# imcbrearty/GENIE

Measured on AMD Instinct MI355X. Metric: picks/sec through GCN_Detection_Network_extended.forward_fixed_source (GCS_Network.forward), higher is better.
Workload: dtype f32

## Files before the change

### genie_amd/_lib.py

```python
import ctypes
import os
import subprocess

_HERE = os.path.dirname(os.path.abspath(__file__))
REPO = os.path.dirname(_HERE)
SRC = os.path.join(_HERE, "csrc", "genie_hip.hip")
LIB_DIR = os.path.join(_HERE, "lib")
LIB_PATH = os.environ.get("GENIE_LIB_PATH", os.path.join(LIB_DIR, "libgenie_hip.so"))
INCLUDE = os.path.join(REPO, "include")

_c = ctypes
_P = _c.c_void_p
SYMBOLS = [
    ("genie_version", _c.c_int, []),
    ("genie_last_error", _c.c_char_p, []),
    ("genie_ctx_create", _c.c_int, [_c.POINTER(_P), _c.c_int, _c.c_int, _c.c_int, _P, _P, _P, _P, _P, _c.c_float]),
    ("genie_ctx_create_subgraph", _c.c_int, [_c.POINTER(_P), _c.c_int, _c.c_int, _c.c_int64, _P, _P, _P, _P, _P, _P, _P, _P, _c.c_float]),
    ("genie_ctx_destroy", _c.c_int, [_P]),
    ("genie_pool_stats", _c.c_int, [_c.c_int, _c.POINTER(_c.c_int64), _c.POINTER(_c.c_int64), _c.POINTER(_c.c_int64)]),
    ("genie_set_scale_t", _c.c_int, [_P, _c.c_float]),
    ("genie_set_edge_features", _c.c_int, [_P, _P, _P, _P]),
    ("genie_set_absolute_pos", _c.c_int, [_P, _P, _P, _P]),
    ("genie_nbr_mean", _c.c_int, [_P, _P, _P, _P, _P, _c.c_int, _P]),
    ("genie_nbr_mean_bwd", _c.c_int, [_P, _P, _P, _P, _P, _c.c_int, _P]),
    ("genie_prelu_bwd", _c.c_int, [_P, _P, _P, _c.c_int64, _P, _P, _P, _P]),
    ("genie_linear_bwd_scratch_floats", _c.c_int64, [_c.c_int]),
    ("genie_linear_bwd_wb", _c.c_int, [_P, _P, _c.c_int64, _c.c_int, _c.c_int, _P, _P, _P, _P]),
    ("genie_set_slot", _c.c_int, [_P, _c.c_int]),
    ("genie_set_station_order", _c.c_int, [_P, _P]),
    ("genie_set_phase_types", _c.c_int, [_P, _c.c_int]),
    ("genie_set_sign_input", _c.c_int, [_P, _c.c_int]),
    ("genie_set_stage2_workmap", _c.c_int, [_P, _c.c_int]),
    ("genie_set_subgraph_stations", _c.c_int, [_P, _P, _P]),
    ("genie_set_tail_precision", _c.c_int, [_P, _c.c_int]),
    ("genie_set_stage_precision", _c.c_int, [_P, _c.c_int]),
    ("genie_stage_precision", _c.c_int, [_P, _c.POINTER(_c.c_int), _c.POINTER(_c.c_int), _c.POINTER(_c.c_float), _c.POINTER(_c.c_float), _P]),
    ("genie_input_range", _c.c_int, [_P, _c.POINTER(_c.c_float), _c.POINTER(_c.c_float), _c.c_int]),
    ("genie_index_flags", _c.c_int, [_P, _c.POINTER(_c.c_uint), _c.c_int]),
    ("genie_index_check", _c.c_int, [_P, _P, _c.c_int64, _c.c_int64, _c.c_int64, _c.c_uint, _P]),
    ("genie_set_static_edge_attr", _c.c_int, [_P, _P, _P]),
    ("genie_tail_batched", _c.c_int, [_P, _c.c_int, _c.c_int, _P, _P, _P, _c.c_int, _c.c_int, _P, _c.c_int, _P, _P, _P, _P, _P]),
    ("genie_readout_grid", _c.c_int, [_P, _P, _P, _c.c_int, _P, _P]),
    ("genie_readout_query", _c.c_int, [_P, _P, _P, _P, _P, _c.c_int, _c.c_int, _P, _c.c_int, _P, _P, _P]),
    ("genie_readouts", _c.c_int, [_P, _P, _P, _P, _P, _c.c_int, _c.c_int, _P, _c.c_int, _P, _P, _P, _P]),
    ("genie_readout_grid_latent", _c.c_int, [_P, _P, _P, _c.c_int, _P, _P, _P]),
    ("genie_readout_query_latent", _c.c_int, [_P, _P, _P, _P, _P, _c.c_int, _c.c_int, _P, _c.c_int, _P, _P, _P, _P]),
    ("genie_weights_count", _c.c_int, []),
    ("genie_weights_name", _c.c_char_p, [_c.c_int]),
    ("genie_weights_numel", _c.c_int64, [_c.c_int]),
    ("genie_weights_offset", _c.c_int64, [_c.c_int]),
    ("genie_weights_blob_floats", _c.c_int64, []),
    ("genie_weights_set", _c.c_int, [_P, _c.c_char_p, _P, _c.c_int64, _P]),
    ("genie_weights_set_blob", _c.c_int, [_P, _P, _c.c_int64, _P]),
    ("genie_weights_commit", _c.c_int, [_P, _P]),
    ("genie_workspace_bytes", _c.c_size_t, [_P]),
# ... 161 lines not shown
```

### genie_amd/csrc/genie_hip.hip

```cpp
#include <hip/hip_runtime.h>
#include <stdint.h>
#include <stdio.h>
#include <stdlib.h>
#include <string.h>

#include <algorithm>
#include <array>
#include <map>
#include <memory>
#include <mutex>
#include <utility>
#include <type_traits>
#include <string>
#include <vector>

#include "genie_hip.h"
#include "s2u_plan.hpp"

#define GENIE_LD_STREAM(ptr) (*(ptr))
#define GENIE_S2_WAVES 2
#define GENIE_H2_DEPTH 6

namespace {

typedef float f32x4 __attribute__((ext_vector_type(4)));

thread_local std::string g_err;

int fail(int code, const std::string& msg) {
    g_err = msg;
    return code;
}

#define HIP_TRY(expr)                                                                              \
    do {                                                                                           \
        hipError_t e_ = (expr);                                                                    \
        if (e_ != hipSuccess)                                                                      \
            return fail(GENIE_ERR_HIP, std::string(#expr) + ": " + hipGetErrorString(e_));         \
    } while (0)
#define GENIE_TRY(expr)                                                                            \
// ... 1092 lines not shown
    int abs_ts_order;
    bool pcsr;
    bool pcsr_h2;
    DevBuf<int32_t> p_sta_rowptr, p_sta_col, p_src_rowptr, p_src_col, seg_rowptr;
    DevBuf<int32_t> p_src_of;
    DevBuf<int32_t> p_sta_of;
    DevBuf<float> mpos_sta, mpos_src, ebias_sta, ebias_src;
    bool has_edges;
    DevBuf<int32_t> sta_perm, sta_inv, sta_rowptr_p, sta_col_p;
    DevBuf<int32_t> sta_ident;
    DevBuf<float> ebias_sta_p;
    const float* ea_user;
    DevBuf<int32_t> src_tab;
    DevBuf<float> packed_h2;
    hipStream_t side_stream;
    hipEvent_t ev_fork, ev_join;
    int device = 0;
    int num_cu;
    int seg, bpc1, bpc2;
    int ks_uni, kp_uni;
    int use_fast;
    int bpc2o;
    int s2_wgmap;
    int bpc1b;
    int use_h2;
    int prec_mode;
    bool range_ok;
    float range_act, range_w;
    DevBuf<float> d_range; float* h_range;
    unsigned* h_inflag;
    struct S2uTables { DevBuf<S2uBlock> blocks; DevBuf<int32_t> xcd0; int nblk, ngroups; };
    std::map<std::pair<int, int>, S2uTables> s2u;
    std::vector<int32_t> tab_host;
    DevBuf<float> packed_s2h;
    DevBuf<unsigned> ea_frag, ea_frag_tmp;
    RowLayout s1_layout;
    std::vector<const void*> lds_attr_done;
    int xs_sta_order;
    int sign_input;
    int no_phase;
    int tail_f32;
    size_t o_xs, o_mm, o_c, o_wu, o_wv, o_part, o_sa0, o_sa1, o_bip, o_gpart, o_pj0, o_pj1, o_cv, ws_floats;
    size_t slot_stride;
    size_t big_stride;
    int tail_cu_ro, tail_cu_sa;
    int slot;
// ... 1004 lines not shown
    }
    return fail(GENIE_ERR_ARG, std::string("genie_weights_set: unknown parameter ") + name);
}

int64_t genie_weights_offset(int i) { init_registry(); return (i >= 0 && i < W_COUNT) ? g_params[i].off : -1; }
int64_t genie_weights_blob_floats(void) { init_registry(); return g_raw_total; }

int genie_weights_set_blob(genie_ctx* c, const float* blob_dev, int64_t n_floats, void* stream) {
    if (!c || !blob_dev) return fail(GENIE_ERR_ARG, "genie_weights_set_blob: null argument");
    if (n_floats != g_raw_total) return fail(GENIE_ERR_ARG, "genie_weights_set_blob: wrong blob size");
    HIP_TRY(hipMemcpyAsync(c->raw, blob_dev, sizeof(float) * n_floats, hipMemcpyDeviceToDevice, (hipStream_t)stream));
    c->dirty = true;
    return GENIE_OK;
}

int genie_weights_commit(genie_ctx* c, void* stream) {
    if (!c) return fail(GENIE_ERR_ARG, "null context");
    return ensure_packed(c, (hipStream_t)stream);
}

size_t genie_workspace_bytes(const genie_ctx* c) { return c ? c->ws_floats * sizeof(float) : 0; }

namespace {
extern "C++" template <bool PCSR>
void launch_stage1_h2(const DaArgs& a, bool abs, bool edges, bool big, int grid, hipStream_t st) {
    if (abs) {
        if (big) k_stage1_h2<8, 15, false, true, true, PCSR><<<grid, H2_THREADS, 0, st>>>(a);
        else k_stage1_h2<8, 15, false, false, true, PCSR><<<grid, H2_THREADS, 0, st>>>(a);
    } else if (edges) {
        if (big) k_stage1_h2<8, 15, true, true, false, PCSR><<<grid, H2_THREADS, 0, st>>>(a);
        else k_stage1_h2<8, 15, true, false, false, PCSR><<<grid, H2_THREADS, 0, st>>>(a);
    } else {
        if (big) k_stage1_h2<8, 15, false, true, false, PCSR><<<grid, H2_THREADS, 0, st>>>(a);
        else k_stage1_h2<8, 15, false, false, false, PCSR><<<grid, H2_THREADS, 0, st>>>(a);
    }
}

int alloc_abs_pieces(genie_ctx* c, size_t n_sta_rows, size_t n_src_rows) {
    DevBuf<unsigned> ts, tg;
    HIP_TRY(ts.alloc(4 * n_sta_rows));
    HIP_TRY(tg.alloc(4 * n_src_rows));
    c->abs_ts = std::move(ts); c->abs_tg = std::move(tg);
    return GENIE_OK;
}

int run_stage1(genie_ctx* c, const StageCall& call, const float* slice, const float* mask, float* dbg_h0, float* dbg_h1, void* ws,
               void* stream, int gi_begin, int gi_end, bool do_split) {
    int rc = check_ws(c, ws);
    if (rc) return rc;
    if (!slice || !mask) return fail(GENIE_ERR_ARG, "genie_da_stage1: null input");
    if (gi_begin < 0 || gi_end > c->G || gi_begin > gi_end) return fail(GENIE_ERR_ARG, "genie_da_stage1: bad source-node range");
    const bool whole = gi_begin == 0 && gi_end == c->G;
    if (!whole && c->pcsr) return fail(GENIE_ERR_STATE, "genie_da_stage1_range: not available on an irregular product graph");
    hipStream_t st = (hipStream_t)stream;
    if ((rc = ensure_packed(c, st))) return rc;
    const StageRoutes r = stage_routes(c, call, gi_begin, gi_end, false, false);
    const bool so = sta_order_on(c, call);
// ... 39 lines not shown
        k_stage1<true><<<(int)std::max<long long>(8, gw / 8 * 8), 256, 0, st>>>(a);
        break;
    }
    case S1Route::H2: {
        unsigned* xs = (unsigned*)((float*)ws + c->o_xs);
        const bool presplit = (c->xs_slice == slice && c->xs_mask == mask && c->xs_ws == ws && c->xs_sta_order == (so ? 1 : 0)) || !do_split;
        if (do_split) { c->xs_slice = c->xs_mask = nullptr; c->xs_ws = nullptr; }
        float* mmw = (float*)ws + c->o_mm + (c->slot % GENIE_NBIG) * c->big_stride;
        if (presplit && do_split && so && c->xs_mm_copy != c->slot % GENIE_NBIG) {
            HIP_TRY(hipMemcpyAsync(mmw, (const float*)ws + c->o_mm + c->xs_mm_copy * c->big_stride, sizeof(float) * (size_t)c->P_ext,
                                   hipMemcpyDeviceToDevice, st));
        }
        if (!presplit) {
            if (so && c->S <= SPLIT_G_MAXS) {
                HIP_TRY(hipFuncSetAttribute((const void*)k_split_rows_g, hipFuncAttributeMaxDynamicSharedMemorySize, SPLIT_G_MAXS * 32));
                k_split_rows_g<<<(unsigned)(c->P_ext / c->S), 256, (size_t)c->S * 32, st>>>(slice, mask, c->S, xs, c->sta_perm, mmw, c->P_ext,
                                                                                            input_limit(c), c->h_inflag);
            } else
                k_split_rows<<<(unsigned)((c->P_ext + 255) / 256), 256, 0, st>>>(slice, mask, c->P_ext, xs, so ? c->sta_perm : nullptr, c->S,
                                                                                mmw, input_limit(c), c->h_inflag);
        }
        a.xs = xs; a.packed = c->packed_h2; a.xs_plane = c->P_ext * (long long)XPC;
        a.np = r.layout == RowLayout::NodePlanar ? 1 : 0;
        const int grid = da_grid_w(c, (n_tiles + 1) / 2, c->bpc1b, H2_THREADS / 64);
        if (!n_tiles) break;
        if (c->abs_sta && (c->abs_dirty || !c->abs_ts || c->abs_ts_order != (so ? 1 : 0))) {
            if (!c->abs_ts) GENIE_TRY(alloc_abs_pieces(c, (size_t)c->S, (size_t)c->G_ext));
            k_abs_pieces<<<(c->S + 255) / 256, 256, 0, st>>>(c->abs_sta, so ? c->sta_perm : nullptr, c->S, c->abs_ts);
            k_abs_pieces<<<(c->G_ext + 255) / 256, 256, 0, st>>>(c->abs_src, nullptr, c->G_ext, c->abs_tg);
            c->abs_dirty = false; c->abs_ts_order = so ? 1 : 0;
            a.abs_ts = c->abs_ts; a.abs_tg = c->abs_tg;
        }
        launch_stage1_h2<false>(a, c->abs_sta != nullptr, c->has_edges, c->P_ext * XROW >= (1ll << 32), grid, st);
        break;
    }
    }
    HIP_TRY(hipGetLastError());
    if (dbg_tmp) {
        if (dbg_h0) k_permute_sta_rows<<<(unsigned)((c->P * 30 + 255) / 256), 256, 0, st>>>(dbg_tmp, c->P, 30, c->sta_perm, c->S, dbg_h0);
        if (dbg_h1) k_permute_sta_rows<<<(unsigned)((c->P * 60 + 255) / 256), 256, 0, st>>>(dbg_tmp + c->P * 30, c->P, 60, c->sta_perm, c->S, dbg_h1);
        HIP_TRY(hipStreamSynchronize(st));
    }
    return GENIE_OK;
}
}

int genie_da_stage1(genie_ctx* c, const float* slice, const float* mask, void* ws, void* stream) {
    if (!c) return fail(GENIE_ERR_ARG, "null context");
    return run_stage1(c, kInference, slice, mask, nullptr, nullptr, ws, stream, 0, c->G, true);
}

int genie_da_stage1_range(genie_ctx* c, const float* slice, const float* mask, int gi_begin, int gi_end, int first, void* ws,
                          void* stream) {
    if (!c) return fail(GENIE_ERR_ARG, "null context");
    return run_stage1(c, kInference, slice, mask, nullptr, nullptr, ws, stream, gi_begin, gi_end, first != 0);
}
// ... 2113 lines not shown
        return fail(GENIE_ERR_ARG, "genie_subgraph_csr_fill: bad argument");
    if (n_prod == 0) return GENIE_OK;
    k_subgraph_csr<true><<<(unsigned)((n_prod + 255) / 256), 256, 0, (hipStream_t)stream>>>(
        pair_sta, pair_src, n_prod, seg_rowptr, sta_rowptr, sta_col, src_rowptr, src_col, nullptr, nullptr, p_sta_rowptr, p_src_rowptr,
        p_sta_col, p_src_col);
    HIP_TRY(hipGetLastError());
    return GENIE_OK;
}

int genie_set_phase_types(genie_ctx* c, int use_phase_types) {
    if (!c) return fail(GENIE_ERR_ARG, "genie_set_phase_types: null context");
    c->no_phase = use_phase_types ? 0 : 1;
    return GENIE_OK;
}

int genie_set_subgraph_stations(genie_ctx* c, const int32_t* sta_of_prod, void* stream) {
    if (!c || !sta_of_prod) return fail(GENIE_ERR_ARG, "genie_set_subgraph_stations: null argument");
    if (!c->pcsr) return fail(GENIE_ERR_STATE, "genie_set_subgraph_stations: the context is a Cartesian product graph (station = p % n_sta)");
    if (!c->p_sta_of) HIP_TRY(c->p_sta_of.alloc((size_t)c->P));
    HIP_TRY(hipMemcpyAsync(c->p_sta_of, sta_of_prod, sizeof(int32_t) * (size_t)c->P, hipMemcpyDeviceToDevice, (hipStream_t)stream));
    return GENIE_OK;
}

int genie_set_stage2_workmap(genie_ctx* c, int blocks_of_four) {
    if (!c) return fail(GENIE_ERR_ARG, "genie_set_stage2_workmap: null context");
    c->s2_wgmap = blocks_of_four < 0 ? (c->S >= 1024) : (blocks_of_four != 0);
    return GENIE_OK;
}

int genie_set_sign_input(genie_ctx* c, int use_sign_input) {
    if (!c) return fail(GENIE_ERR_ARG, "genie_set_sign_input: null context");
    c->sign_input = use_sign_input ? 1 : 0;
    return GENIE_OK;
}

int genie_set_tail_precision(genie_ctx* c, int fp64_chains) {
    if (!c) return fail(GENIE_ERR_ARG, "genie_set_tail_precision: null context");
    c->tail_f32 = fp64_chains ? 0 : 1;
    return GENIE_OK;
}

int genie_set_stage_precision(genie_ctx* c, int mode) {
    if (!c || mode < 0 || mode > 2) return fail(GENIE_ERR_ARG, "genie_set_stage_precision: mode must be 0 (auto), 1 (f16x2) or 2 (fp32)");
    c->prec_mode = mode;
    c->xs_slice = c->xs_mask = nullptr; c->xs_ws = nullptr;
    return GENIE_OK;
// ... 65 lines not shown
```

### genie_amd/csrc/stage_kernels.hpp

```cpp

template <int N>
__device__ __forceinline__ void mma_blocks(f32x4 (&acc)[N], const f32x4 (&w)[N], const f32x4 x) {
#pragma unroll
    for (int r = 0; r < 4; ++r) {
#pragma unroll
        for (int k = 0; k < N; ++k) acc[k] = MFMA16(w[k][r], x[r], acc[k]);
    }
}

__device__ __forceinline__ void stage1_dense(const DaArgs& a, const f32x4* lw, const float* lbias, int lane, int q,
                                             bool valid, long long p, int g, int sc, float mq, f32x4 x0, f32x4 x1, f32x4 n1a,
                                             f32x4 n1b, f32x4 n2a, f32x4 n2b, float a1, float a21, float a22) {
    if (a.dbg_h0 != nullptr && valid) {
#pragma unroll
        for (int r = 0; r < 4; ++r) {
            a.dbg_h0[p * 30 + 4 * q + r] = x0[r];
            if (16 + 4 * q + r < 30) a.dbg_h0[p * 30 + 16 + 4 * q + r] = x1[r];
        }
    }
    f32x4 acc[4], w4[4];
#pragma unroll
    for (int k = 0; k < 4; ++k) acc[k] = *(const f32x4*)(lbias + (2 + k) * 16 + 4 * q);
    if (a.eb_sta != nullptr) {
#pragma unroll
// ... 342 lines not shown
        const f32x4 t = *(const f32x4*)(lbias + blk * 32 + 8 * b + 4 * h);
        y[4 * b] = t.x; y[4 * b + 1] = t.y; y[4 * b + 2] = t.z; y[4 * b + 3] = t.w;
    }
    return y;
}
__device__ __forceinline__ void h2_save32(float* __restrict__ save, long long Pn, int blk0, long long p, int h, const f32x16& v) {
#pragma unroll
    for (int m = 0; m < 4; ++m) {
        f32x4 o = {v[4 * m], v[4 * m + 1], v[4 * m + 2], v[4 * m + 3]};
        if (m == 3 && h == 1) { o.z = 0.f; o.w = 0.f; }
        *(f32x4*)(save + ((size_t)(blk0 + (m >> 1)) * Pn + p) * 16 + 8 * (m & 1) + 4 * h) = o;
    }
}
template <int K_>
__device__ __forceinline__ int row_bcast(int v) { return __builtin_amdgcn_update_dpp(0, v, 0x150 + K_, 0xf, 0xf, false); }
__device__ __forceinline__ int row_bcast_dyn(int v, int k) {
    switch (k) {
        case 0: return row_bcast<0>(v); case 1: return row_bcast<1>(v); case 2: return row_bcast<2>(v); case 3: return row_bcast<3>(v);
        case 4: return row_bcast<4>(v); case 5: return row_bcast<5>(v); case 6: return row_bcast<6>(v); case 7: return row_bcast<7>(v);
        case 8: return row_bcast<8>(v); case 9: return row_bcast<9>(v); case 10: return row_bcast<10>(v); case 11: return row_bcast<11>(v);
        case 12: return row_bcast<12>(v); case 13: return row_bcast<13>(v); case 14: return row_bcast<14>(v); default: return row_bcast<15>(v);
    }
}
template <int KS_>
__device__ __forceinline__ void split8h(const f32x16& v, u32x4 (&p)[3], unsigned sixteenth) {
#pragma unroll
    for (int d = 0; d < 4; ++d) {
        const float a = v[8 * KS_ + 2 * d], b = v[8 * KS_ + 2 * d + 1];
        const unsigned p0 = cvt_pk_f16(a, b);
        p[0][d] = p0;
        p[1][d] = cvt_pk_f16(sub_f16_lo(a, p0), sub_f16_hi(b, p0));
        p[2][d] = pk_mul_f16(p0, sixteenth);
    }
}
template <int N>
__device__ __forceinline__ void mma3(f32x16 (&acc)[N], const f32x4* lw, const int (&f0)[N], int lane, const u32x4 (&b)[3]) {
    f32x4 w[N][2];
#pragma unroll
    for (int k = 0; k < N; ++k)
#pragma unroll
        for (int p = 0; p < 2; ++p) w[k][p] = lw[(f0[k] + p) * 64 + lane];
    constexpr int WP[3] = {0, 1, 0}, BP[3] = {1, 2, 0};
#pragma unroll
    for (int t = 0; t < 3; ++t)
#pragma unroll
        for (int k = 0; k < N; ++k) acc[k] = MFMA32H(w[k][WP[t]], b[BP[t]], acc[k]);
}

#ifndef GENIE_S1_NT_C
#define GENIE_S1_NT_C 1
#endif
__device__ __forceinline__ void h2_store_c(f32x4* p, f32x4 v) {
#if GENIE_S1_NT_C
    __builtin_nontemporal_store(v, p);
#else
    *p = v;
#endif
}

template <int KS, int KP, bool EDGES, bool BIG, bool ABS = false, bool PCSR = false>
__global__ __launch_bounds__(H2_THREADS) void k_stage1_h2(DaArgs a) {
    typedef typename std::conditional<BIG, unsigned long long, unsigned>::type off_t_;
    constexpr int NF4 = H2_IMG_FLOATS / 4;
    __shared__ f32x4 lw[NF4];
    for (int i = threadIdx.x; i < NF4; i += H2_THREADS) lw[i] = ((const f32x4*)a.packed)[i];
    __syncthreads();
    const float* lbias = (const float*)(lw + H2_FRAGS * 64);
    const float* lscal = lbias + H2_NBIAS * 32;
    const float a0 = lscal[0], a1 = lscal[3], a21 = lscal[4], a22 = lscal[5];
    const float s11 = compose_slopes(a0, lscal[1]), s12 = compose_slopes(a0, lscal[2]);
    const float inf = __builtin_inff();
    const float sel0 = a0 <= 1.f ? inf : -inf, sel1 = a1 <= 1.f ? inf : -inf;
    const float sel21 = a21 <= 1.f ? inf : -inf, sel22 = a22 <= 1.f ? inf : -inf;
    const float al1 = (1.f + s11) / (32.f * KS), be1 = (1.f - s11) / (32.f * KS);
    const float al2 = (1.f + s12) / (32.f * KP), be2 = (1.f - s12) / (32.f * KP);
    const unsigned c16 = __builtin_amdgcn_readfirstlane(H2_SIXTEENTH);

    int lane = threadIdx.x & 63;
    const int wave = __builtin_amdgcn_readfirstlane(threadIdx.x >> 6);
    const int h = lane >> 5, half = (lane >> 4) & 1, jj = lane & 15;
    const bool hi = h != 0;
    const int S = a.S;
    ItemIter w(a.G, a.T, a.seg, a.nxcd, wave, a.gi0);
    const char* xs = (const char*)a.xs;
    const off_t_ la = hi ? (off_t_)a.xs_plane : (off_t_)0;
    const off_t_ gstride = (off_t_)((unsigned)S * (unsigned)XPC);

    const f32x4 fa0 = lw[(H2_FA + 0) * 64 + lane], fa1 = lw[(H2_FA + 1) * 64 + lane];
    f32x4 fp0, fp1;
    if (ABS) { fp0 = lw[(H2_FABS + 0) * 64 + lane]; fp1 = lw[(H2_FABS + 1) * 64 + lane]; }
    const unsigned tp_h = (unsigned)h * 8u;
    typedef unsigned u32x2 __attribute__((ext_vector_type(2)));
    f32x16 biasA = bias16(lbias, 0, h);
#pragma unroll
    for (int r = 0; r < 16; ++r) biasA[r] *= 16.f;

    int jt = jj;
    auto fetch_ids = [&](long long pit_, int& idv_, int& sc_, bool& valid_, int (&sta_)[KS]) {
        int gi0, tb0, gi1, tb1;
        w.decode(2 * pit_, gi0, tb0);
        const bool second = 2 * pit_ + 1 < w.nitems;
        w.decode(second ? 2 * pit_ + 1 : 2 * pit_, gi1, tb1);
        idv_ = a.src_tab[(half ? gi1 : gi0) * 16 + jt];
        const int s = (half ? tb1 : tb0) * 16 + jt;
        valid_ = s < S && (second || !half);
        sc_ = s < S ? s : S - 1;
        load_sta_ids<KS>(a.sta_col, sc_, sta_);
    };
    constexpr int KPP = PCSR ? KP : 1;
    auto fetch_pcsr = [&](long long pit_, long long& p_, bool& valid_, int (&sta_)[KS], int (&src_)[KPP], int& ds_, int& dp_) {
        const long long pr = ptile_at(a.ptile, pit_) * 32 + (lane & 31);
        valid_ = pr < a.Pn;
        p_ = valid_ ? pr : a.Pn - 1;
        const int eb = a.sta_rowptr[p_], fb = a.src_rowptr[p_];
        ds_ = a.sta_rowptr[p_ + 1] - eb;
        dp_ = a.src_rowptr[p_ + 1] - fb;
#pragma unroll
        for (int q = 0; q < KS; ++q) {
            const int v = a.sta_col[max(eb + min(q, ds_ - 1), 0)];
            sta_[q] = q < ds_ ? v : (int)p_;
        }
#pragma unroll
        for (int q = 0; q < KPP; ++q) {
            const int v = a.src_col[max(fb + min(q, dp_ - 1), 0)];
            src_[q] = q < dp_ ? v : (int)p_;
        }
    };
    int idv = 0, sc = 0, sta_id[KS], src_id[KPP], dgs = 0, dgp = 0;
    long long pcur = 0;
    bool valid = false;
    PtileIter ptw(PCSR ? (a.Pn + 31) / 32 : 0, H2_THREADS / 64, wave);
    const long long pit0 = PCSR ? ptw.i : w.it;
    const long long pstride = PCSR ? ptw.stride : w.stride;
    const long long pend = PCSR ? ptw.end : (w.nitems + 1) / 2;
    if (pit0 < pend) {
        if constexpr (PCSR) fetch_pcsr(pit0, pcur, valid, sta_id, src_id, dgs, dgp);
        else fetch_ids(pit0, idv, sc, valid, sta_id);
    }
    for (long long pit = pit0, pnext = 0; pit < pend; pit = pnext) {
        asm volatile("" : "+v"(lane));
        const int g = PCSR ? 0 : row_bcast<0>(idv);
        const long long p = PCSR ? pcur : (long long)g * S + sc;
        const off_t_ gbase0 = PCSR ? (off_t_)(unsigned long long)p * (off_t_)XPC : (off_t_)(unsigned)g * gstride;
        const unsigned sbase0 = PCSR ? 0u : (unsigned)sc * (unsigned)XPC;
        off_t_ gbase = gbase0 + la;
        off_t_ sbase = (off_t_)sbase0 + la;
        const int srcv = idv;
        float alS = 0.f, beS = 0.f, alP = 0.f, beP = 0.f;
        if constexpr (PCSR) {
            const float is = 1.f / (float)max(dgs, 1), ip = 1.f / (float)max(dgp, 1);
            alS = (1.f + s11) * 0.03125f * is; beS = (1.f - s11) * 0.03125f * is;
            alP = (1.f + s12) * 0.03125f * ip; beP = (1.f - s12) * 0.03125f * ip;
        }

        constexpr int NU = 1 + KS + KP;
        static_assert(NU % 2 == 0, "units are processed in pairs");
        constexpr int DEPTH = ABS ? 4 : GENIE_H2_DEPTH;
        u32x4 buf[NU];
        u32x2 tp[NU], tso, tgo;
        if (ABS) {
            tso = *(const u32x2*)((const char*)a.abs_ts + (tp_h + (unsigned)(PCSR ? (int)p : sc) * 16u));
            tgo = *(const u32x2*)((const char*)a.abs_tg + (tp_h + (unsigned)(PCSR ? (int)p : g) * 16u));
        }
        auto issue = [&](int u) {
            off_t_ off;
            if (u == 0) off = gbase + sbase0;
            else if (PCSR) off = (off_t_)(unsigned)(u <= KS ? sta_id[u - 1] : src_id[(u - KS - 1) % KPP]) * (off_t_)XPC + la;
            else if (u <= KS) off = gbase + (unsigned)sta_id[u - 1] * (unsigned)XPC;
            else {
                const unsigned nb = (unsigned)row_bcast_dyn(srcv, u - KS);
                off = (BIG ? (off_t_)nb * gstride : (off_t_)__umul24(nb, (unsigned)gstride)) + sbase;
            }
            if (ABS && u > 0) {
                if (u <= KS) tp[u] = *(const u32x2*)((const char*)a.abs_ts + (tp_h + (unsigned)sta_id[u - 1] * 16u));
                else if (PCSR) tp[u] = *(const u32x2*)((const char*)a.abs_tg + (tp_h + (unsigned)src_id[(u - KS - 1) % KPP] * 16u));
                else tp[u] = *(const u32x2*)((const char*)a.abs_tg + (tp_h + (unsigned)row_bcast_dyn(srcv, u - KS) * 16u));
            }
            buf[u] = *(const u32x4*)(xs + off);
        };
        const u32x4 own0 = *(const u32x4*)(xs + (gbase0 + sbase0));
#pragma unroll
        for (int u = 0; u < DEPTH; ++u) issue(u);

        f32x16 sn, h0;
        u32x4 h0p[2][3], n1p[2][3], n2p[2][3];
        unsigned m01[3], m23[3];
#pragma unroll
        for (int u = 0; u < NU; u += 2) {
#pragma unroll
            for (int d = 0; d < 2; ++d)
                if (u + DEPTH + d < NU) issue(u + DEPTH + d);
            asm volatile("" : "+v"(buf[u]), "+v"(buf[u + 1]));
            f32x16 z0, z1;
            if (ABS) {
                auto posb = [&](int uu) {
                    return uu == 0 ? u32x4{tso.x, tso.y, tgo.x, tgo.y}
                                   : uu <= KS ? u32x4{tp[uu].x, tp[uu].y, tgo.x, tgo.y} : u32x4{tso.x, tso.y, tp[uu].x, tp[uu].y};
                };
                const u32x4 p0 = posb(u), p1 = posb(u + 1);
// ... 22 lines not shown
                    m01[0] = own0.z;   m23[0] = own0.w;
                    m01[1] = buf[0].z; m23[1] = buf[0].w;
                    m01[2] = pk_mul_f16(own0.z, c16); m23[2] = pk_mul_f16(own0.w, c16);
                } else {
                    float al = uu <= KS ? al1 : al2, be = uu <= KS ? be1 : be2;
                    if constexpr (PCSR) {
                        const bool present = uu <= KS ? uu - 1 < dgs : uu - KS - 1 < dgp;
                        al = present ? (uu <= KS ? alS : alP) : 0.f;
                        be = present ? (uu <= KS ? beS : beP) : 0.f;
                    }
                    if (uu == 1 || uu == KS + 1) {
#pragma unroll
                        for (int r = 0; r < 16; ++r) sn[r] = fmaf(be, __builtin_fabsf(z[r]), al * z[r]);
                    } else {
#pragma unroll
                        for (int r = 0; r < 16; ++r) sn[r] = fmaf(be, __builtin_fabsf(z[r]), fmaf(al, z[r], sn[r]));
                    }
                }
                if (uu == KS) { split8h<0>(sn, n1p[0], c16); split8h<1>(sn, n1p[1], c16); }
                if (uu == NU - 1) { split8h<0>(sn, n2p[0], c16); split8h<1>(sn, n2p[1], c16); }
            }
            asm volatile("" : "+v"(sn), "+v"(gbase), "+v"(sbase), "+v"(jt));
        }
        int idv_n = 0, sc_n = 0, sta_n[KS], src_n[KPP], dgs_n = 0, dgp_n = 0;
        long long p_n = 0;
        bool valid_n = false;
#pragma unroll
        for (int k = 0; k < KS; ++k) sta_n[k] = 0;
#pragma unroll
        for (int k = 0; k < KPP; ++k) src_n[k] = 0;
        pnext = pit + pstride;
        const bool has_next = pnext < pend;
        if (has_next) {
            if constexpr (PCSR) fetch_pcsr(pnext, p_n, valid_n, sta_n, src_n, dgs_n, dgp_n);
            else fetch_ids(pnext, idv_n, sc_n, valid_n, sta_n);
        }
        if (a.dbg_h0 != nullptr && valid) {
#pragma unroll
            for (int r = 0; r < 16; ++r) {
                const int ch = 8 * (r >> 2) + 4 * h + (r & 3);
                if (ch < 30) a.dbg_h0[p * 30 + ch] = h0[r];
            }
        }
        split8h<0>(h0, h0p[0], c16);
        split8h<1>(h0, h0p[1], c16);
#pragma unroll
        for (int q = 0; q < 3; ++q) {
            h0p[1][q].w = hi ? m01[q] : h0p[1][q].w;
            n1p[1][q].w = hi ? m23[q] : n1p[1][q].w;
            n2p[1][q].w = hi ? m23[q] : n2p[1][q].w;
        }
        f32x16 acc[2] = {bias16(lbias, 1, h), bias16(lbias, 2, h)};
        if (EDGES) {
#pragma unroll
            for (int b = 0; b < 4; ++b) {
                const f32x4 es = *(const f32x4*)(a.eb_sta + (PCSR ? p : (long long)sc) * 48 + 8 * b + 4 * h);
                const f32x4 eg = *(const f32x4*)(a.eb_src + (PCSR ? p : (long long)g) * 48 + 8 * b + 4 * h);
#pragma unroll
// ... 78 lines not shown
            else { split8h<1>(o3[0], up, c16); split8h<1>(o3[1], vp, c16); }
            f32x4 wa[2], wb[2];
#pragma unroll
            for (int q = 0; q < 2; ++q) {
                wa[q] = lw[(H2_FW + (0 + kb) * 2 + q) * 64 + lane];
                wb[q] = lw[(H2_FW + (2 + kb) * 2 + q) * 64 + lane];
            }
            constexpr int WP[3] = {0, 1, 0}, BP[3] = {1, 2, 0};
#pragma unroll
            for (int t = 0; t < 3; ++t) {
                ow[0] = MFMA32H(wa[WP[t]], up[BP[t]], ow[0]);
                ow[1] = MFMA32H(wb[WP[t]], vp[BP[t]], ow[1]);
            }
        }
        if (valid) {
            float* vr = a.np ? a.wv + npb * ROWW + (long long)h * npl + (long long)sc * 4 : a.wv + p * ROWW + 4 * h;
            const long long vs = a.np ? 2 * npl : 8;
#pragma unroll
            for (int b = 0; b < 2; ++b) {
                *(f32x4*)(a.wu + p * ROWW + 8 * b + 4 * h) = f32x4{ow[0][4 * b], ow[0][4 * b + 1], ow[0][4 * b + 2], ow[0][4 * b + 3]};
                *(f32x4*)(vr + b * vs) = f32x4{ow[1][8 + 4 * b], ow[1][8 + 4 * b + 1], ow[1][8 + 4 * b + 2], ow[1][8 + 4 * b + 3]};
            }
        }
        idv = idv_n; sc = sc_n; valid = valid_n; pcur = p_n; dgs = dgs_n; dgp = dgp_n;
#pragma unroll
        for (int k = 0; k < KS; ++k) sta_id[k] = sta_n[k];
#pragma unroll
        for (int k = 0; k < KPP; ++k) src_id[k] = src_n[k];
    }
}

template <bool UNI>
__device__ __forceinline__ void stage2_row_sums(const DaArgs& a, long long pc, int qc, const float* wu0, const float* wv0,
                                                long long wv_stride, int eb1, int ee1, int eb2, int ee2, f32x4 (&o)[2]) {
    o[0] = *(const f32x4*)(a.c + pc * ROWC + 4 * qc);
    o[1] = *(const f32x4*)(a.c + pc * ROWC + 16 + 4 * qc);
    f32x4 n1 = {0.f, 0.f, 0.f, 0.f}, n2 = {0.f, 0.f, 0.f, 0.f};
    gather_sum16<false>(wu0 + 4 * qc, ROWW, a.sta_col, eb1, ee1, n1);
    o[0] = fma4(n1, 1.f / (float)max(ee1 - eb1, 1), o[0]);
    gather_sum16<UNI>(wv0 + 4 * qc, wv_stride, a.src_col, eb2, ee2, n2);
    o[1] = fma4(n2, 1.f / (float)max(ee2 - eb2, 1), o[1]);
}

__device__ __forceinline__ void stage2_x_latent(const DaArgs& a, bool valid, long long pc, int qc, float a2, f32x4 (&o)[2]) {
    if (a.save != nullptr && valid) {
        *(f32x4*)(a.save + ((size_t)(SV_O + 0) * a.Pn + pc) * 16 + 4 * qc) = o[0];
        *(f32x4*)(a.save + ((size_t)(SV_O + 1) * a.Pn + pc) * 16 + 4 * qc) = o[1];
// ... 717 lines not shown
```

### genie_amd/engine.py

```python
import ctypes
import os

import numpy as np
import torch

from . import _lib


def _ptr(t):
    return ctypes.c_void_p(t.data_ptr()) if t is not None else ctypes.c_void_p(0)


def _stream():
    return ctypes.c_void_p(torch.cuda.current_stream().cuda_stream)


def _f32(t, name, shape=None):
    if not torch.is_tensor(t):
        raise TypeError("%s must be a torch tensor" % name)
    if not t.is_cuda:
        raise ValueError("%s must live on the GPU (got %s); the HIP path has no CPU fallback" % (name, t.device))
    if t.dtype != torch.float32:
        t = t.float()
    t = t.contiguous()
# ... 620 lines not shown
            n = self.lib.genie_weights_count()
            HipPath._registry = ([self.lib.genie_weights_name(i).decode() for i in range(n)],
                                 [int(self.lib.genie_weights_numel(i)) for i in range(n)],
                                 [int(self.lib.genie_weights_offset(i)) for i in range(n)], int(self.lib.genie_weights_blob_floats()))
        self.w_names, self.w_numel, self.w_off, n_blob = HipPath._registry
        self._blob = torch.zeros(n_blob, dtype=torch.float32, device=dev)
        self._w_key = None

    _registry = None

    def set_subgraph_stations(self, sta_of_prod):
        if self._n_prod is None:
            raise ValueError("set_subgraph_stations: not an irregular product graph")
        t = torch.as_tensor(sta_of_prod).to(self.device, torch.int32).contiguous()
        if t.numel() != self._n_prod:
            raise ValueError("sta_of_prod must have n_prod entries")
        _lib.check(self.lib.genie_set_subgraph_stations(self.ctx, _ptr(t), _stream()), "genie_set_subgraph_stations")
        torch.cuda.current_stream().synchronize()

    def set_stage2_workmap(self, blocks_of_four):
        v = -1 if blocks_of_four is None else (1 if blocks_of_four else 0)
        _lib.check(self.lib.genie_set_stage2_workmap(self.ctx, v), "genie_set_stage2_workmap")

    def set_sign_input(self, use_sign_input):
        _lib.check(self.lib.genie_set_sign_input(self.ctx, 1 if use_sign_input else 0), "genie_set_sign_input")

    def set_phase_types(self, use_phase_types):
        _lib.check(self.lib.genie_set_phase_types(self.ctx, 1 if use_phase_types else 0), "genie_set_phase_types")

    def set_tail_precision(self, fp64_chains):
        _lib.check(self.lib.genie_set_tail_precision(self.ctx, 1 if fp64_chains else 0), "genie_set_tail_precision")

    def set_stage_precision(self, mode):
        if mode not in _PRECISION_MODES:
            raise ValueError("stage_precision must be one of %s" % (sorted(_PRECISION_MODES),))
        _lib.check(self.lib.genie_set_stage_precision(self.ctx, _PRECISION_MODES[mode]), "genie_set_stage_precision")

    def stage_precision(self):
        mode, act = ctypes.c_int(0), ctypes.c_int(0)
        ab, wb = ctypes.c_float(0), ctypes.c_float(0)
        _lib.check(self.lib.genie_stage_precision(self.ctx, ctypes.byref(mode), ctypes.byref(act), ctypes.byref(ab), ctypes.byref(wb),
                                                  _stream()), "genie_stage_precision")
        names = {v: k for k, v in _PRECISION_MODES.items()}
        return {"mode": names[mode.value], "f16x2_active": bool(act.value), "act_bound": float(ab.value), "weight_bound": float(wb.value)}

    def __del__(self):
# ... 875 lines not shown
```

### include/genie_hip.h

```cpp
#ifndef GENIE_HIP_H
#define GENIE_HIP_H

#include <stddef.h>
#include <stdint.h>

#ifdef __cplusplus
extern "C" {
#endif

typedef struct genie_ctx genie_ctx;

#define GENIE_OK 0
#define GENIE_ERR_ARG (-1)
#define GENIE_ERR_HIP (-2)
#define GENIE_ERR_STATE (-3)

int genie_version(void);
const char* genie_last_error(void);

int genie_ctx_create(genie_ctx** out, int n_sta, int n_grid, int n_grid_ext,
                     const int32_t* sta_rowptr, const int32_t* sta_col,
                     const int32_t* src_rowptr, const int32_t* src_col,
                     const int32_t* grid_order, float scale_rel);
int genie_ctx_create_subgraph(genie_ctx** out, int n_sta, int n_grid, int64_t n_prod,
                              const int32_t* p_sta_rowptr, const int32_t* p_sta_col,
                              const int32_t* p_src_rowptr, const int32_t* p_src_col, const int32_t* seg_rowptr,
                              const int32_t* src_rowptr, const int32_t* src_col, const int32_t* grid_order, float scale_rel);
int genie_set_subgraph_stations(genie_ctx* ctx, const int32_t* sta_of_prod, void* stream);
int genie_ctx_destroy(genie_ctx* ctx);
int genie_pool_stats(int device, int64_t* live_blocks, int64_t* live_bytes, int64_t* cached_bytes);
int genie_set_station_order(genie_ctx* ctx, const int32_t* order);
int genie_set_phase_types(genie_ctx* ctx, int use_phase_types);
int genie_set_sign_input(genie_ctx* ctx, int use_sign_input);
int genie_set_stage2_workmap(genie_ctx* ctx, int blocks_of_four);
int genie_set_tail_precision(genie_ctx* ctx, int fp64_chains);
int genie_set_stage_precision(genie_ctx* ctx, int mode);
int genie_stage_precision(genie_ctx* ctx, int* mode, int* f16x2_active, float* act_bound, float* weight_bound, void* stream);
int genie_input_range(genie_ctx* ctx, float* max_seen, float* limit, int reset);
int genie_index_flags(genie_ctx* ctx, unsigned* flags, int reset);
int genie_index_check(genie_ctx* ctx, const int64_t* idx, int64_t n, int64_t lo, int64_t hi, unsigned bit, void* stream);
int genie_set_static_edge_attr(genie_ctx* ctx, const float* edge_attr, void* stream);
int genie_set_slot(genie_ctx* ctx, int slot);
int genie_tail_batched(genie_ctx* ctx, int slot0, int nwin, const float* pos, const float* x_query, const int32_t* knn,
                       int n_query, int k, const float* t_query, int n_t, float* x_spatial_out, float* y_out, float* x_out,
                       void* ws, void* stream);
int genie_set_scale_t(genie_ctx* ctx, float scale_t);
int genie_set_absolute_pos(genie_ctx* ctx, const float* pos_sta, const float* pos_src, void* stream);
int genie_set_edge_features(genie_ctx* ctx, const float* pos_sta, const float* pos_src, void* stream);

int genie_weights_count(void);
const char* genie_weights_name(int i);
int64_t genie_weights_numel(int i);
int64_t genie_weights_offset(int i);
int64_t genie_weights_blob_floats(void);
int genie_weights_set(genie_ctx* ctx, const char* name, const float* dev_ptr, int64_t numel, void* stream);
int genie_weights_set_blob(genie_ctx* ctx, const float* blob_dev, int64_t n_floats, void* stream);
int genie_weights_commit(genie_ctx* ctx, void* stream);
// ... 245 lines not shown
```

Before: 87.85 million.

## Pack half-empty tail station tiles of two grid nodes into one work item

When the station count leaves a final 16-lane tile that is at most half full, stage-1 work items now pair the tail tiles of two neighbouring grid nodes. Each pair shares one 16-lane item, with 8 lanes per node, and a second source-id register is merged in through DPP row broadcasts. A new item decoder in tile_items.hpp enumerates the mixed items, which cuts the number of items by about G/2 and reduces idle lanes. The cost is extra decode arithmetic, an extra src_tab load and extra DPP ops per item. A new setter allows turning the packing off.

```diff
diff --git a/genie_amd/_lib.py b/genie_amd/_lib.py
--- a/genie_amd/_lib.py
+++ b/genie_amd/_lib.py
@@ -31,6 +31,7 @@
     ("genie_set_phase_types", _c.c_int, [_P, _c.c_int]),
     ("genie_set_sign_input", _c.c_int, [_P, _c.c_int]),
     ("genie_set_stage2_workmap", _c.c_int, [_P, _c.c_int]),
+    ("genie_set_tail_packing", _c.c_int, [_P, _c.c_int]),
     ("genie_set_subgraph_stations", _c.c_int, [_P, _P, _P]),
     ("genie_set_tail_precision", _c.c_int, [_P, _c.c_int]),
     ("genie_set_stage_precision", _c.c_int, [_P, _c.c_int]),
diff --git a/genie_amd/csrc/genie_hip.hip b/genie_amd/csrc/genie_hip.hip
--- a/genie_amd/csrc/genie_hip.hip
+++ b/genie_amd/csrc/genie_hip.hip
@@ -16,6 +16,7 @@
 
 #include "genie_hip.h"
 #include "s2u_plan.hpp"
+#include "tile_items.hpp"
 
 #define GENIE_LD_STREAM(ptr) (*(ptr))
 #define GENIE_S2_WAVES 2
@@ -1154,6 +1155,7 @@
     int use_fast;
     int bpc2o;
     int s2_wgmap;
+    bool no_tail_pack;
     int bpc1b;
     int use_h2;
     int prec_mode;
@@ -2204,17 +2206,17 @@
 size_t genie_workspace_bytes(const genie_ctx* c) { return c ? c->ws_floats * sizeof(float) : 0; }
 
 namespace {
-extern "C++" template <bool PCSR>
+extern "C++" template <bool PCSR, bool MIX = false>
 void launch_stage1_h2(const DaArgs& a, bool abs, bool edges, bool big, int grid, hipStream_t st) {
     if (abs) {
-        if (big) k_stage1_h2<8, 15, false, true, true, PCSR><<<grid, H2_THREADS, 0, st>>>(a);
-        else k_stage1_h2<8, 15, false, false, true, PCSR><<<grid, H2_THREADS, 0, st>>>(a);
+        if (big) k_stage1_h2<8, 15, false, true, true, PCSR, MIX><<<grid, H2_THREADS, 0, st>>>(a);
+        else k_stage1_h2<8, 15, false, false, true, PCSR, MIX><<<grid, H2_THREADS, 0, st>>>(a);
     } else if (edges) {
-        if (big) k_stage1_h2<8, 15, true, true, false, PCSR><<<grid, H2_THREADS, 0, st>>>(a);
-        else k_stage1_h2<8, 15, true, false, false, PCSR><<<grid, H2_THREADS, 0, st>>>(a);
+        if (big) k_stage1_h2<8, 15, true, true, false, PCSR, MIX><<<grid, H2_THREADS, 0, st>>>(a);
+        else k_stage1_h2<8, 15, true, false, false, PCSR, MIX><<<grid, H2_THREADS, 0, st>>>(a);
     } else {
-        if (big) k_stage1_h2<8, 15, false, true, false, PCSR><<<grid, H2_THREADS, 0, st>>>(a);
-        else k_stage1_h2<8, 15, false, false, false, PCSR><<<grid, H2_THREADS, 0, st>>>(a);
+        if (big) k_stage1_h2<8, 15, false, true, false, PCSR, MIX><<<grid, H2_THREADS, 0, st>>>(a);
+        else k_stage1_h2<8, 15, false, false, false, PCSR, MIX><<<grid, H2_THREADS, 0, st>>>(a);
     }
 }
 
@@ -2300,7 +2302,9 @@
         }
         a.xs = xs; a.packed = c->packed_h2; a.xs_plane = c->P_ext * (long long)XPC;
         a.np = r.layout == RowLayout::NodePlanar ? 1 : 0;
-        const int grid = da_grid_w(c, (n_tiles + 1) / 2, c->bpc1b, H2_THREADS / 64);
+        const bool mix = tile_items::packs(c->S) && !c->no_tail_pack;
+        const long long n_items = mix ? n_tiles - a.G / 2 : n_tiles;
+        const int grid = da_grid_w(c, (n_items + 1) / 2, c->bpc1b, H2_THREADS / 64);
         if (!n_tiles) break;
         if (c->abs_sta && (c->abs_dirty || !c->abs_ts || c->abs_ts_order != (so ? 1 : 0))) {
             if (!c->abs_ts) GENIE_TRY(alloc_abs_pieces(c, (size_t)c->S, (size_t)c->G_ext));
@@ -2309,7 +2313,8 @@
             c->abs_dirty = false; c->abs_ts_order = so ? 1 : 0;
             a.abs_ts = c->abs_ts; a.abs_tg = c->abs_tg;
         }
-        launch_stage1_h2<false>(a, c->abs_sta != nullptr, c->has_edges, c->P_ext * XROW >= (1ll << 32), grid, st);
+        if (mix) launch_stage1_h2<false, true>(a, c->abs_sta != nullptr, c->has_edges, c->P_ext * XROW >= (1ll << 32), grid, st);
+        else launch_stage1_h2<false>(a, c->abs_sta != nullptr, c->has_edges, c->P_ext * XROW >= (1ll << 32), grid, st);
         break;
     }
     }
@@ -4469,6 +4474,12 @@
     return GENIE_OK;
 }
 
+int genie_set_tail_packing(genie_ctx* c, int on) {
+    if (!c) return fail(GENIE_ERR_ARG, "genie_set_tail_packing: null context");
+    c->no_tail_pack = on == 0;
+    return GENIE_OK;
+}
+
 int genie_set_stage2_workmap(genie_ctx* c, int blocks_of_four) {
     if (!c) return fail(GENIE_ERR_ARG, "genie_set_stage2_workmap: null context");
     c->s2_wgmap = blocks_of_four < 0 ? (c->S >= 1024) : (blocks_of_four != 0);
diff --git a/genie_amd/csrc/stage_kernels.hpp b/genie_amd/csrc/stage_kernels.hpp
--- a/genie_amd/csrc/stage_kernels.hpp
+++ b/genie_amd/csrc/stage_kernels.hpp
@@ -388,6 +388,16 @@
         case 12: return row_bcast<12>(v); case 13: return row_bcast<13>(v); case 14: return row_bcast<14>(v); default: return row_bcast<15>(v);
     }
 }
+template <int K_>
+__device__ __forceinline__ int row_bcast_hi(int lo, int hi) { return __builtin_amdgcn_update_dpp(lo, hi, 0x150 + K_, 0xf, 0xc, false); }
+__device__ __forceinline__ int row_bcast_hi_dyn(int lo, int hi, int k) {
+    switch (k) {
+        case 0: return row_bcast_hi<0>(lo, hi); case 1: return row_bcast_hi<1>(lo, hi); case 2: return row_bcast_hi<2>(lo, hi); case 3: return row_bcast_hi<3>(lo, hi);
+        case 4: return row_bcast_hi<4>(lo, hi); case 5: return row_bcast_hi<5>(lo, hi); case 6: return row_bcast_hi<6>(lo, hi); case 7: return row_bcast_hi<7>(lo, hi);
+        case 8: return row_bcast_hi<8>(lo, hi); case 9: return row_bcast_hi<9>(lo, hi); case 10: return row_bcast_hi<10>(lo, hi); case 11: return row_bcast_hi<11>(lo, hi);
+        case 12: return row_bcast_hi<12>(lo, hi); case 13: return row_bcast_hi<13>(lo, hi); case 14: return row_bcast_hi<14>(lo, hi); default: return row_bcast_hi<15>(lo, hi);
+    }
+}
 template <int KS_>
 __device__ __forceinline__ void split8h(const f32x16& v, u32x4 (&p)[3], unsigned sixteenth) {
 #pragma unroll
@@ -424,8 +434,9 @@
 #endif
 }
 
-template <int KS, int KP, bool EDGES, bool BIG, bool ABS = false, bool PCSR = false>
+template <int KS, int KP, bool EDGES, bool BIG, bool ABS = false, bool PCSR = false, bool MIX = false>
 __global__ __launch_bounds__(H2_THREADS) void k_stage1_h2(DaArgs a) {
+    static_assert(!(MIX && PCSR), "an irregular product graph has no station tiles");
     typedef typename std::conditional<BIG, unsigned long long, unsigned>::type off_t_;
     constexpr int NF4 = H2_IMG_FLOATS / 4;
     __shared__ f32x4 lw[NF4];
@@ -448,6 +459,9 @@
     const bool hi = h != 0;
     const int S = a.S;
     ItemIter w(a.G, a.T, a.seg, a.nxcd, wave, a.gi0);
+    tile_items::Packed wp;
+    if constexpr (MIX) wp.init(w.gbeg, w.gend, a.T, a.seg);
+    const long long nitems = MIX ? wp.nitems : w.nitems;
     const char* xs = (const char*)a.xs;
     const off_t_ la = hi ? (off_t_)a.xs_plane : (off_t_)0;
     const off_t_ gstride = (off_t_)((unsigned)S * (unsigned)XPC);
@@ -462,13 +476,23 @@
     for (int r = 0; r < 16; ++r) biasA[r] *= 16.f;
 
     int jt = jj;
-    auto fetch_ids = [&](long long pit_, int& idv_, int& sc_, bool& valid_, int (&sta_)[KS]) {
-        int gi0, tb0, gi1, tb1;
-        w.decode(2 * pit_, gi0, tb0);
-        const bool second = 2 * pit_ + 1 < w.nitems;
-        w.decode(second ? 2 * pit_ + 1 : 2 * pit_, gi1, tb1);
+    auto fetch_ids = [&](long long pit_, int& idv_, int& idw_, int& sc_, bool& valid_, int (&sta_)[KS]) {
+        int gi0, tb0, gi1, tb1, gj0 = 0, gj1 = 0;
+        const bool second = 2 * pit_ + 1 < nitems;
+        if constexpr (MIX) {
+            wp.decode(2 * pit_, gi0, gj0, tb0);
+            wp.decode(second ? 2 * pit_ + 1 : 2 * pit_, gi1, gj1, tb1);
+        } else {
+            w.decode(2 * pit_, gi0, tb0);
+            w.decode(second ? 2 * pit_ + 1 : 2 * pit_, gi1, tb1);
+        }
         idv_ = a.src_tab[(half ? gi1 : gi0) * 16 + jt];
-        const int s = (half ? tb1 : tb0) * 16 + jt;
+        int js = jt;
+        if constexpr (MIX) {
+            idw_ = a.src_tab[(half ? gj1 : gj0) * 16 + jt];
+            js = (half ? gj1 != gi1 : gj0 != gi0) ? (jt & 7) : jt;
+        }
+        const int s = (half ? tb1 : tb0) * 16 + js;
         valid_ = s < S && (second || !half);
         sc_ = s < S ? s : S - 1;
         load_sta_ids<KS>(a.sta_col, sc_, sta_);
@@ -492,26 +516,32 @@
             src_[q] = q < dp_ ? v : (int)p_;
         }
     };
-    int idv = 0, sc = 0, sta_id[KS], src_id[KPP], dgs = 0, dgp = 0;
+    int idv = 0, idw = 0, sc = 0, sta_id[KS], src_id[KPP], dgs = 0, dgp = 0;
     long long pcur = 0;
     bool valid = false;
     PtileIter ptw(PCSR ? (a.Pn + 31) / 32 : 0, H2_THREADS / 64, wave);
     const long long pit0 = PCSR ? ptw.i : w.it;
     const long long pstride = PCSR ? ptw.stride : w.stride;
-    const long long pend = PCSR ? ptw.end : (w.nitems + 1) / 2;
+    const long long pend = PCSR ? ptw.end : (nitems + 1) / 2;
     if (pit0 < pend) {
         if constexpr (PCSR) fetch_pcsr(pit0, pcur, valid, sta_id, src_id, dgs, dgp);
-        else fetch_ids(pit0, idv, sc, valid, sta_id);
+        else fetch_ids(pit0, idv, idw, sc, valid, sta_id);
     }
     for (long long pit = pit0, pnext = 0; pit < pend; pit = pnext) {
         asm volatile("" : "+v"(lane));
-        const int g = PCSR ? 0 : row_bcast<0>(idv);
+        int g = PCSR ? 0 : row_bcast<0>(idv);
+        if constexpr (MIX) g = row_bcast_hi<0>(g, idw);
         const long long p = PCSR ? pcur : (long long)g * S + sc;
         const off_t_ gbase0 = PCSR ? (off_t_)(unsigned long long)p * (off_t_)XPC : (off_t_)(unsigned)g * gstride;
         const unsigned sbase0 = PCSR ? 0u : (unsigned)sc * (unsigned)XPC;
         off_t_ gbase = gbase0 + la;
         off_t_ sbase = (off_t_)sbase0 + la;
-        const int srcv = idv;
+        const int srcv = idv, srcw = idw;
+        auto src_nb = [&](int k) {
+            int nb = row_bcast_dyn(srcv, k);
+            if constexpr (MIX) nb = row_bcast_hi_dyn(nb, srcw, k);
+            return (unsigned)nb;
+        };
         float alS = 0.f, beS = 0.f, alP = 0.f, beP = 0.f;
         if constexpr (PCSR) {
             const float is = 1.f / (float)max(dgs, 1), ip = 1.f / (float)max(dgp, 1);
@@ -534,13 +564,13 @@
             else if (PCSR) off = (off_t_)(unsigned)(u <= KS ? sta_id[u - 1] : src_id[(u - KS - 1) % KPP]) * (off_t_)XPC + la;
             else if (u <= KS) off = gbase + (unsigned)sta_id[u - 1] * (unsigned)XPC;
             else {
-                const unsigned nb = (unsigned)row_bcast_dyn(srcv, u - KS);
+                const unsigned nb = src_nb(u - KS);
                 off = (BIG ? (off_t_)nb * gstride : (off_t_)__umul24(nb, (unsigned)gstride)) + sbase;
             }
             if (ABS && u > 0) {
                 if (u <= KS) tp[u] = *(const u32x2*)((const char*)a.abs_ts + (tp_h + (unsigned)sta_id[u - 1] * 16u));
                 else if (PCSR) tp[u] = *(const u32x2*)((const char*)a.abs_tg + (tp_h + (unsigned)src_id[(u - KS - 1) % KPP] * 16u));
-                else tp[u] = *(const u32x2*)((const char*)a.abs_tg + (tp_h + (unsigned)row_bcast_dyn(srcv, u - KS) * 16u));
+                else tp[u] = *(const u32x2*)((const char*)a.abs_tg + (tp_h + src_nb(u - KS) * 16u));
             }
             buf[u] = *(const u32x4*)(xs + off);
         };
@@ -609,7 +639,7 @@
             }
             asm volatile("" : "+v"(sn), "+v"(gbase), "+v"(sbase), "+v"(jt));
         }
-        int idv_n = 0, sc_n = 0, sta_n[KS], src_n[KPP], dgs_n = 0, dgp_n = 0;
+        int idv_n = 0, idw_n = 0, sc_n = 0, sta_n[KS], src_n[KPP], dgs_n = 0, dgp_n = 0;
         long long p_n = 0;
         bool valid_n = false;
 #pragma unroll
@@ -620,7 +650,7 @@
         const bool has_next = pnext < pend;
         if (has_next) {
             if constexpr (PCSR) fetch_pcsr(pnext, p_n, valid_n, sta_n, src_n, dgs_n, dgp_n);
-            else fetch_ids(pnext, idv_n, sc_n, valid_n, sta_n);
+            else fetch_ids(pnext, idv_n, idw_n, sc_n, valid_n, sta_n);
         }
         if (a.dbg_h0 != nullptr && valid) {
 #pragma unroll
@@ -745,7 +775,7 @@
                 *(f32x4*)(vr + b * vs) = f32x4{ow[1][8 + 4 * b], ow[1][8 + 4 * b + 1], ow[1][8 + 4 * b + 2], ow[1][8 + 4 * b + 3]};
             }
         }
-        idv = idv_n; sc = sc_n; valid = valid_n; pcur = p_n; dgs = dgs_n; dgp = dgp_n;
+        idv = idv_n; idw = idw_n; sc = sc_n; valid = valid_n; pcur = p_n; dgs = dgs_n; dgp = dgp_n;
 #pragma unroll
         for (int k = 0; k < KS; ++k) sta_id[k] = sta_n[k];
 #pragma unroll
diff --git a/genie_amd/csrc/tile_items.hpp b/genie_amd/csrc/tile_items.hpp
--- /dev/null
+++ b/genie_amd/csrc/tile_items.hpp
@@ -0,0 +1,80 @@
+#pragma once
+#include <cstdint>
+
+#if defined(__HIPCC__)
+#define TILE_ITEMS_HD __host__ __device__ __forceinline__
+#else
+#define TILE_ITEMS_HD inline
+#endif
+
+namespace tile_items {
+
+TILE_ITEMS_HD bool packs(int S) { return (S & 15) >= 1 && (S & 15) <= 8; }
+
+TILE_ITEMS_HD void chunk(int gi0, int G, int x, int nx, int& gbeg, int& gend) {
+    gbeg = gi0 + (int)((long long)G * x / nx);
+    gend = gi0 + (int)((long long)G * (x + 1) / nx);
+}
+
+TILE_ITEMS_HD long long count(int n, int T, int seg) {
+    if (seg <= 1) return (long long)(n / 2) * (2 * T - 1) + (long long)(n & 1) * T;
+    const int full = n / seg, rest = n - full * seg;
+    return (long long)full * ((long long)seg * (T - 1) + (seg + 1) / 2) + (long long)rest * (T - 1) + (rest + 1) / 2;
+}
+
+struct Packed {
+    int gbeg, T;
+    unsigned seg, per, m_per, n_full, m_full, n_last, m_last, last_seg;
+    long long nitems;
+    static TILE_ITEMS_HD unsigned fdiv(unsigned x, unsigned d, unsigned m, unsigned& r) {
+        unsigned q = (unsigned)(((unsigned long long)x * m) >> 32);
+        r = x - q * d;
+        if (r >= d) { r -= d; ++q; }
+        if (r >= d) { r -= d; ++q; }
+        return q;
+    }
+    static TILE_ITEMS_HD unsigned recip(unsigned d) { return d <= 1u ? 0xffffffffu : (unsigned)(0x100000000ull / d); }
+    TILE_ITEMS_HD void init(int gbeg_, int gend_, int T_, int seg_) {
+        gbeg = gbeg_; T = T_;
+        const int n = gend_ - gbeg_;
+        seg = (unsigned)(seg_ <= 1 ? 1 : seg_);
+        const unsigned span = seg == 1u ? 2u : seg;
+        per = seg == 1u ? (unsigned)(2 * T - 1) : seg * (unsigned)(T - 1) + (seg + 1u) / 2u;
+        m_per = recip(per);
+        n_full = span; m_full = recip(n_full);
+        last_seg = (unsigned)n / span;
+        n_last = (unsigned)n - last_seg * span;
+        if (n_last == 0u) n_last = 1u;
+        m_last = recip(n_last);
+        nitems = count(n, T, (int)seg);
+    }
+    TILE_ITEMS_HD void decode(long long item, int& gi, int& gj, int& tb) const {
+        unsigned rem, r2;
+        const unsigned sidx = per <= 1u ? (rem = 0u, (unsigned)item) : fdiv((unsigned)item, per, m_per, rem);
+        const bool last = sidx >= last_seg;
+        const unsigned tm1 = (unsigned)(T - 1);
+        if (seg == 1u) {
+            const int base = gbeg + 2 * (int)sidx;
+            const bool second = !last && rem > tm1;
+            gi = base + (second ? 1 : 0);
+            gj = gi + ((!last && rem == tm1) ? 1 : 0);
+            tb = (int)(second ? rem - tm1 - 1u : rem);
+            return;
+        }
+        const unsigned n = last ? n_last : n_full;
+        const unsigned nt = n * tm1;
+        const int base = gbeg + (int)(sidx * seg);
+        if (rem < nt) {
+            const unsigned q = n <= 1u ? (r2 = 0u, rem) : fdiv(rem, n, last ? m_last : m_full, r2);
+            tb = (int)q;
+            gi = gj = base + (int)r2;
+        } else {
+            const unsigned j = rem - nt;
+            tb = (int)tm1;
+            gi = base + 2 * (int)j;
+            gj = gi + (2u * j + 1u < n ? 1 : 0);
+        }
+    }
+};
+
+}
diff --git a/genie_amd/engine.py b/genie_amd/engine.py
--- a/genie_amd/engine.py
+++ b/genie_amd/engine.py
@@ -666,6 +666,9 @@
         v = -1 if blocks_of_four is None else (1 if blocks_of_four else 0)
         _lib.check(self.lib.genie_set_stage2_workmap(self.ctx, v), "genie_set_stage2_workmap")
 
+    def set_tail_packing(self, on):
+        _lib.check(self.lib.genie_set_tail_packing(self.ctx, 1 if on else 0), "genie_set_tail_packing")
+
     def set_sign_input(self, use_sign_input):
         _lib.check(self.lib.genie_set_sign_input(self.ctx, 1 if use_sign_input else 0), "genie_set_sign_input")
 
diff --git a/include/genie_hip.h b/include/genie_hip.h
--- a/include/genie_hip.h
+++ b/include/genie_hip.h
@@ -33,6 +33,7 @@
 int genie_set_phase_types(genie_ctx* ctx, int use_phase_types);
 int genie_set_sign_input(genie_ctx* ctx, int use_sign_input);
 int genie_set_stage2_workmap(genie_ctx* ctx, int blocks_of_four);
+int genie_set_tail_packing(genie_ctx* ctx, int on);
 int genie_set_tail_precision(genie_ctx* ctx, int fp64_chains);
 int genie_set_stage_precision(genie_ctx* ctx, int mode);
 int genie_stage_precision(genie_ctx* ctx, int* mode, int* f16x2_active, float* act_bound, float* weight_bound, void* stream);
```

Measured after the change: 88.85 million (median of 6 runs). 1.1% higher.
